# akashsengupta1997/STRAPS-3DHumanShapePose

Hardware: AMD Instinct MI355X
Metric: bodies/sec (higher is better)
Workload: dtype fp32 (encoder convolutions as exact bf16x3 operand splits (six bf16 products per term); in-step SMPL blend contraction and skinning as 3-product fp16 splits (fp16x3_lbs: 22-bit operands); fp32 accumulate throughout)

## Files before the change

straps-3dhumanshapepose_amd/csrc/elementwise.hip:

```cpp
#include "common.h"

namespace {

__global__ __launch_bounds__(256) void pack_krsc_kernel(const float* __restrict__ src, float* __restrict__ dst, int O, int C, int R, int S) {
    const long long i = (long long)blockIdx.x * 256 + threadIdx.x;
    const long long n = (long long)O * C * R * S;
    if (i >= n) return;
    const int c = (int)(i % C);
    long long t = i / C;
    const int s = (int)(t % S); t /= S;
    const int r = (int)(t % R);
    const int o = (int)(t / R);
    dst[i] = src[(((long long)o * C + c) * R + r) * S + s];
}

__global__ __launch_bounds__(256) void pack_crsk_flip_kernel(const float* __restrict__ src, float* __restrict__ dst, int O, int C, int R, int S) {
    const long long i = (long long)blockIdx.x * 256 + threadIdx.x;
    const long long n = (long long)O * C * R * S;
    if (i >= n) return;
    const int o = (int)(i % O);
    long long t = i / O;
    const int s = (int)(t % S); t /= S;
    const int r = (int)(t % R);
    const int c = (int)(t / R);
// ... 145 lines not shown
                const f32x4 v = *reinterpret_cast<const f32x4*>(x + (((long long)b * H + hi) * W + wi) * C + c4 * 4);
                m[0] = fmaxf(m[0], v[0]); m[1] = fmaxf(m[1], v[1]); m[2] = fmaxf(m[2], v[2]); m[3] = fmaxf(m[3], v[3]);
            }
        }
        *reinterpret_cast<f32x4*>(y + i * 4) = m;
    }
}

__global__ __launch_bounds__(256) void gap_kernel(const float* __restrict__ x, float* __restrict__ y, int B, int HW, int C) {
    const long long i = (long long)blockIdx.x * 256 + threadIdx.x;
    if (i >= (long long)B * C) return;
    const int c = (int)(i % C);
    const long long b = i / C;
    const float* p = x + b * HW * C + c;
    float s = 0.f;
    for (int k = 0; k < HW; ++k) s += p[(long long)k * C];
    y[i] = s / (float)HW;
}

__global__ __launch_bounds__(256) void bn_stats_finalize_kernel(const float* __restrict__ part, int nblocks, int C, double count,
                                                               const float* __restrict__ gamma, const float* __restrict__ beta, float eps,
                                                               float momentum, float* __restrict__ rmean, float* __restrict__ rvar,
                                                               float* __restrict__ scale, float* __restrict__ shift,
                                                               float* __restrict__ smean, float* __restrict__ sinv) {
    int c;
    double s1, s2;
    if (bn_partials_sum4(part, nblocks, C, s1, s2, c)) {
        const double mean = s1 / count;
        double var = s2 / count - mean * mean;
        if (var < 0.0) var = 0.0;
        const float inv = (float)(1.0 / sqrt(var + (double)eps));
// ... 193 lines not shown
```

straps-3dhumanshapepose_amd/csrc/smpl_bwd.hip:

```cpp
#include "common.h"
#include "rodrigues.h"

namespace {

constexpr int KP = STRAPS_SMPL_KP, KG = KP / 8, NT = STRAPS_SMPL_TILES, NV = STRAPS_SMPL_V, NROUNDS = NT / 4;
constexpr int BT = 32, AS = 292, SS = 193;
constexpr int NJS = STRAPS_SMPL_NPICK + STRAPS_SMPL_NEXTRA;

__global__ __launch_bounds__(256, 1) STRAPS_NO_PACKED_FP32 void smpl_verts_bwd_kernel(straps_smpl_model_t m, const float* __restrict__ F,
                                                                const float* __restrict__ Amat, const float* __restrict__ dverts,
                                                                const float* __restrict__ djoints, float* __restrict__ dFp,
                                                                float* __restrict__ dAp, long long B, int rounds_per_chunk) {
    extern __shared__ __attribute__((aligned(16))) float smem[];
    float* As_ = smem;
    float* stage = As_ + BT * AS;

    const int tid = threadIdx.x, lane = tid & 63, wave = tid >> 6;
    const int h = lane >> 5, bl = lane & 31;
    const int chunk = blockIdx.x;
    const long long b0 = (long long)blockIdx.y * BT;
    const int nb = (int)((B - b0) < BT ? (B - b0) : BT);

    for (int i = tid; i < BT * 72; i += 256) {
        const int b = i / 72, q = i % 72;
        f32x4 v = {0.f, 0.f, 0.f, 0.f};
        if (b < nb) v = *reinterpret_cast<const f32x4*>(Amat + (b0 + b) * 288 + q * 4);
        *reinterpret_cast<f32x4*>(As_ + b * AS + q * 4) = v;
    }
    __syncthreads();

    const int round0 = chunk * rounds_per_chunk;
    const int round1 = min(round0 + rounds_per_chunk, NROUNDS);
    const f32x4* __restrict__ blend = reinterpret_cast<const f32x4*>(m.blend_frag);
    const f32x4* __restrict__ blend_t = reinterpret_cast<const f32x4*>(m.blend_frag_t);
    float* mystage = stage + wave * BT * SS;
    const int KW = m.skin_k;
    const bool vbody = bl < nb;

    float dacc[3][12];
#pragma unroll
    for (int i = 0; i < 3; ++i)
#pragma unroll
        for (int e = 0; e < 12; ++e) dacc[i][e] = 0.f;
    f32x16 accF[7];
#pragma unroll
    for (int f = 0; f < 7; ++f)
#pragma unroll
        for (int q = 0; q < 16; ++q) accF[f][q] = 0.f;

    for (int rd = round0; rd < round1; ++rd) {
        const int tile = rd * 4 + wave;
        f32x16 ax, ay, az;
#pragma unroll
        for (int r = 0; r < 16; ++r) { ax[r] = 0.f; ay[r] = 0.f; az[r] = 0.f; }
        {
            const f32x4* px = blend + ((long long)(tile * 3 + 0) * KG) * 64 + lane;
            const f32x4* py = px + KG * 64;
            const f32x4* pz = py + KG * 64;
            const float* frow = F + (b0 + (vbody ? bl : 0)) * KP + 4 * h;
            f32x4 cx0 = px[0], cy0 = py[0], cz0 = pz[0];
            f32x4 fn = *reinterpret_cast<const f32x4*>(frow);
#pragma unroll 2
            for (int g = 0; g < KG; ++g) {
                f32x4 nx0 = cx0, ny0 = cy0, nz0 = cz0;
                const f32x4 f0 = vbody ? fn : f32x4{0.f, 0.f, 0.f, 0.f};
                if (g + 1 < KG) {
                    nx0 = px[(g + 1) * 64]; ny0 = py[(g + 1) * 64]; nz0 = pz[(g + 1) * 64];
                    fn = *reinterpret_cast<const f32x4*>(frow + 8 * (g + 1));
                }
#pragma unroll
                for (int e = 0; e < 4; ++e) {
                    ax = mfma32(cx0[e], f0[e], ax);
                    ay = mfma32(cy0[e], f0[e], ay);
                    az = mfma32(cz0[e], f0[e], az);
                }
                cx0 = nx0; cy0 = ny0; cz0 = nz0;
            }
        }
        {
            const int ncol = min(96, (NV - tile * 32) * 3);
            for (int i = lane; i < BT * 96; i += 64) {
                const int b = i / 96, c = i - b * 96;
                float v = 0.f;
                if (dverts && b < nb && c < ncol) v = dverts[(b0 + b) * (long long)(NV * 3) + tile * 96 + c];
                mystage[b * SS + (c / 3) * 6 + (c % 3)] = v;
            }
        }
        __syncthreads();
        if (djoints && h == 0 && vbody) {
            const float* dj = djoints + (b0 + bl) * (STRAPS_SMPL_NJOINTS_OUT * 3) + 72;
            const int e0 = m.jrt_ptr[tile], e1 = m.jrt_ptr[tile + 1];
            for (int e = e0; e < e1; ++e) {
                const int code = m.jrt_code[e];
                const float w = m.jrt_w[e];
                float* sv = mystage + bl * SS + (code >> 8) * 6;
                const float* g = dj + (code & 255) * 3;
                sv[0] = fmaf(w, g[0], sv[0]); sv[1] = fmaf(w, g[1], sv[1]); sv[2] = fmaf(w, g[2], sv[2]);
            }
        }
        __syncthreads();
        {
            const float* Ab = As_ + bl * AS;
#pragma unroll
            for (int r = 0; r < 16; ++r) {
                const int vrow = (r & 3) + 8 * (r >> 2) + 4 * h;
                const int v = tile * 32 + vrow;
                float* sv = mystage + bl * SS + vrow * 6;
                const float gx = sv[0], gy = sv[1], gz = sv[2];
                sv[3] = ax[r]; sv[4] = ay[r]; sv[5] = az[r];
                float t00 = 0.f, t01 = 0.f, t02 = 0.f, t10 = 0.f, t11 = 0.f, t12 = 0.f, t20 = 0.f, t21 = 0.f, t22 = 0.f;
                for (int k = 0; k < KW; ++k) {
                    const float w = m.skin_w[v * KW + k];
                    const int jo = m.skin_j[v * KW + k] * 12;
                    const f32x4 a0 = *reinterpret_cast<const f32x4*>(Ab + jo);
                    const f32x4 a1 = *reinterpret_cast<const f32x4*>(Ab + jo + 4);
                    const f32x4 a2 = *reinterpret_cast<const f32x4*>(Ab + jo + 8);
                    t00 += w * a0[0]; t01 += w * a0[1]; t02 += w * a0[2];
                    t10 += w * a1[0]; t11 += w * a1[1]; t12 += w * a1[2];
                    t20 += w * a2[0]; t21 += w * a2[1]; t22 += w * a2[2];
                }
                ax[r] = t00 * gx + t10 * gy + t20 * gz;
                ay[r] = t01 * gx + t11 * gy + t21 * gz;
                az[r] = t02 * gx + t12 * gy + t22 * gz;
            }
        }
        __syncthreads();
#pragma unroll
        for (int i = 0; i < 3; ++i) {
            const int j = wave + 4 * (2 * i + h);
            const int e0 = m.dj_ptr[rd * 24 + j], e1 = m.dj_ptr[rd * 24 + j + 1];
            for (int e = e0; e < e1; ++e) {
                const int code = m.dj_code[e];
                const float w = m.dj_w[e];
                const float* sv = stage + ((code >> 5) * BT + bl) * SS + (code & 31) * 6;
                const float wx = w * sv[0], wy = w * sv[1], wz = w * sv[2];
                const float x = sv[3], y = sv[4], z = sv[5];
                dacc[i][0] = fmaf(wx, x, dacc[i][0]); dacc[i][1] = fmaf(wx, y, dacc[i][1]); dacc[i][2] = fmaf(wx, z, dacc[i][2]); dacc[i][3] += wx;
                dacc[i][4] = fmaf(wy, x, dacc[i][4]); dacc[i][5] = fmaf(wy, y, dacc[i][5]); dacc[i][6] = fmaf(wy, z, dacc[i][6]); dacc[i][7] += wy;
                dacc[i][8] = fmaf(wz, x, dacc[i][8]); dacc[i][9] = fmaf(wz, y, dacc[i][9]); dacc[i][10] = fmaf(wz, z, dacc[i][10]); dacc[i][11] += wz;
            }
        }
        {
            const f32x4* pt = blend_t + ((long long)tile * 3 * 7 * 4) * 64 + lane;
#pragma unroll
            for (int c = 0; c < 3; ++c) {
#pragma unroll
                for (int f = 0; f < 7; ++f) {
#pragma unroll
                    for (int rq = 0; rq < 4; ++rq) {
                        const f32x4 a = pt[((c * 7 + f) * 4 + rq) * 64];
#pragma unroll
                        for (int e = 0; e < 4; ++e) {
                            const float g = c == 0 ? ax[rq * 4 + e] : (c == 1 ? ay[rq * 4 + e] : az[rq * 4 + e]);
                            accF[f] = mfma32(a[e], g, accF[f]);
                        }
                    }
                }
            }
        }
        __syncthreads();
    }
    {
        __syncthreads();
        float* red = smem;
        if (wave >= 2) {
#pragma unroll
            for (int f = 0; f < 7; ++f)
#pragma unroll
                for (int q = 0; q < 16; ++q) red[(wave - 2) * 7168 + (f * 16 + q) * 64 + lane] = accF[f][q];
        }
        __syncthreads();
// ... 25 lines not shown
#pragma unroll
            for (int q = 0; q < 16; ++q) o[f * 32 + mfma_row(q, lane)] = accF[f][q];
    }
    if (vbody) {
        float* o = dAp + ((long long)chunk * B + b0 + bl) * 288;
#pragma unroll
        for (int i = 0; i < 3; ++i) {
            const int j = wave + 4 * (2 * i + h);
#pragma unroll
            for (int e = 0; e < 12; ++e) o[j * 12 + e] = dacc[i][e];
        }
    }
}

__device__ __forceinline__ float lane_get(float value, int src) { return __shfl(value, src, 64); }
template <bool AA>
__global__ __launch_bounds__(256) STRAPS_NO_PACKED_FP32 void smpl_pose_bwd_kernel(straps_smpl_model_t m, const float* __restrict__ betas,
                                                            const float* __restrict__ rotmats, const float* __restrict__ dFp,
                                                            const float* __restrict__ dAp, const float* __restrict__ djoints,
                                                            float* __restrict__ dbetas, float* __restrict__ drot, long long B,
                                                            int chunks, const float* __restrict__ aa, float* __restrict__ daa) {
    const int lane = threadIdx.x & 63;
    const int j = lane & 31;
    const int base = lane & 32;
    const long long body = ((long long)blockIdx.x * 256 + threadIdx.x) >> 5;
    const bool vb = body < B;
    const bool vj = j < 24;
    const long long bb = vb ? body : 0;
    const int jj = vj ? j : 0;

// ... 35 lines not shown
#pragma unroll
            for (int r = 0; r < 3; ++r) {
                const float p0 = P[r * 4 + 0], p1 = P[r * 4 + 1], p2 = P[r * 4 + 2];
                PR[r * 3 + 0] = p0; PR[r * 3 + 1] = p1; PR[r * 3 + 2] = p2;
                G[r * 4 + 0] = p0 * R[0] + p1 * R[3] + p2 * R[6];
                G[r * 4 + 1] = p0 * R[1] + p1 * R[4] + p2 * R[7];
                G[r * 4 + 2] = p0 * R[2] + p1 * R[5] + p2 * R[8];
                G[r * 4 + 3] = p0 * rel[0] + p1 * rel[1] + p2 * rel[2] + P[r * 4 + 3];
            }
        }
    }
    float gA[12];
#pragma unroll
    for (int e = 0; e < 12; ++e) gA[e] = 0.f;
    if (vb && vj)
        for (int c = 0; c < chunks; ++c) {
            const float* p = dAp + (((long long)c * B + body) * 24 + j) * 12;
#pragma unroll
            for (int e = 0; e < 12; ++e) gA[e] += p[e];
        }
    float gGR[9], gGt[3], gJ[3];
#pragma unroll
    for (int r = 0; r < 3; ++r) {
        const float gat = gA[r * 4 + 3];
        gGR[r * 3 + 0] = gA[r * 4 + 0] - gat * J[0];
        gGR[r * 3 + 1] = gA[r * 4 + 1] - gat * J[1];
        gGR[r * 3 + 2] = gA[r * 4 + 2] - gat * J[2];
        gGt[r] = gat + ((vb && vj && djoints) ? djoints[(body * STRAPS_SMPL_NJOINTS_OUT + j) * 3 + r] : 0.f);
    }
#pragma unroll
    for (int c = 0; c < 3; ++c) gJ[c] = -(G[0 * 4 + c] * gA[3] + G[1 * 4 + c] * gA[7] + G[2 * 4 + c] * gA[11]);

    int child[3];
#pragma unroll
// ... 34 lines not shown
#pragma unroll
                for (int e = 0; e < 9; ++e) gGR[e] += in[e];
#pragma unroll
                for (int c = 0; c < 3; ++c) { gGt[c] += in[9 + c]; gJ[c] += in[12 + c]; }
            }
        }
    }
    if (j == 0) {
#pragma unroll
        for (int e = 0; e < 9; ++e) gR[e] = gGR[e];
#pragma unroll
        for (int c = 0; c < 3; ++c) gJ[c] += gGt[c];
    }
    float gbeta_direct = 0.f;
    if (vb && vj) {
        for (int c = 0; c < chunks; ++c) {
            const float* p = dFp + ((long long)c * B + body) * KP;
            if (j >= 1) {
#pragma unroll
                for (int e = 0; e < 9; ++e) gR[e] += p[11 + (j - 1) * 9 + e];
            }
            if (j < 10) gbeta_direct += p[1 + j];
        }
        if (!AA || drot) {
#pragma unroll
            for (int e = 0; e < 9; ++e) drot[(body * 24 + j) * 9 + e] = gR[e];
        }
        if constexpr (AA) {
            float ox, oy, oz;
            const float* r = aa + (body * 24 + j) * 3;
            straps_rodrigues_bwd_one(r[0], r[1], r[2], gR, ox, oy, oz);
            float* o = daa + (body * 24 + j) * 3;
            o[0] = ox; o[1] = oy; o[2] = oz;
        }
    }
#pragma unroll
    for (int l = 0; l < 10; ++l) {
// ... 25 lines not shown

namespace {
template <bool AA>
int smpl_bwd_launch(const straps_smpl_model_t* model, const float* betas, const float* rotmats, const float* aa, const float* dverts,
                    const float* djoints, float* dbetas, float* drotmats, float* daa, void* workspace, long long batch, int chunks,
                    void* stream) {
    hipStream_t st = (hipStream_t)stream;
    const int rpc = resolve_rpc(batch, chunks);
    const int nch = (NROUNDS + rpc - 1) / rpc;
    float* F = (float*)workspace;
    float* Amat = F + batch * KP;
    float* dFp = Amat + batch * 288;
    float* dAp = dFp + (long long)nch * batch * KP;
    int rc = straps_smpl_launch_pose(model, betas, rotmats, F, Amat, nullptr, batch, st);
    if (rc != STRAPS_OK) return rc;
    const size_t lds = (size_t)(BT * AS + 4 * BT * SS) * sizeof(float);
    STRAPS_RAISE_LDS((smpl_verts_bwd_kernel), lds, "smpl_verts_bwd_kernel");
    const long long btiles = (batch + BT - 1) / BT;
    if (btiles > 65535) { straps_set_error("straps_smpl_bwd: batch %lld exceeds one launch; split it", batch); return STRAPS_EUNSUPPORTED; }
    hipLaunchKernelGGL(smpl_verts_bwd_kernel, dim3(nch, (unsigned)btiles), dim3(256), lds, st, *model, F, Amat, dverts, djoints, dFp, dAp, batch, rpc);
    STRAPS_CHECK_LAUNCH("smpl_verts_bwd_kernel");
    hipLaunchKernelGGL(smpl_pose_bwd_kernel<AA>, dim3((unsigned)((batch * 32 + 255) / 256)), dim3(256), 0, st, *model, betas, rotmats, dFp, dAp,
                       djoints, dbetas, drotmats, batch, nch, aa, daa);
    STRAPS_CHECK_LAUNCH("smpl_pose_bwd_kernel");
    return STRAPS_OK;
}
}

extern "C" int straps_smpl_bwd(const straps_smpl_model_t* model, const float* betas, const float* rotmats, const float* dverts,
                               const float* djoints, float* dbetas, float* drotmats, void* workspace, long long batch, int chunks,
                               void* stream) {
// ... 18 lines not shown
```

straps-3dhumanshapepose_amd/csrc/train.hip:

```cpp
#include <math.h>

#include "common.h"

namespace {

__constant__ int c_coco[17] = {24, 26, 25, 28, 27, 16, 17, 18, 19, 20, 21, 1, 2, 4, 5, 7, 8};
__constant__ int c_h36m14[14] = {73 + 6, 73 + 5, 73 + 4, 73 + 1, 73 + 2, 73 + 3, 73 + 16, 73 + 15, 73 + 14, 73 + 11, 73 + 12, 73 + 13, 73 + 8, 73 + 10};

__device__ __forceinline__ float heat_value(int x, int y, int jx, int jy, int WH, int size, float step, float two_var) {
    if (!(jx > -size && jy > -size && jx < WH - 1 + size && jy < WH - 1 + size)) return 0.f;
    const int hx0 = max(0, jx - size), hx1 = min(WH - 1, jx + size);
    const int hy0 = max(0, jy - size), hy1 = min(WH - 1, jy + size);
    if (!(x >= hx0 && x < hx1 && y >= hy0 && y < hy1)) return 0.f;
    const int gx = x - hx0 + max(0, size - jx), gy = y - hy0 + max(0, size - jy);
    const float fs = (float)size;
    const float lx = gx < size ? -fs + step * gx : fs - step * (2 * size - 1 - gx);
    const float ly = gy < size ? -fs + step * gy : fs - step * (2 * size - 1 - gy);
    const float d = sqrtf(lx * lx + ly * ly);
    return expf(-(d * d / two_var));
}

__global__ __launch_bounds__(256) void build_proxy_kernel(const float* __restrict__ seg, const float* __restrict__ j2d,
                                                          float* __restrict__ out, int B, int NJ, int WH, int size, float step, float two_var) {
    const int plane = blockIdx.y;
// ... 69 lines not shown
            }
        }
#pragma unroll
        for (int r = 0; r < 4; ++r)
            if (y0 + r < WH) {
                *reinterpret_cast<f32x4*>(o + (y0 + r) * WH + x0) = v[r];
                nz = nz || v[r][0] != 0.f || v[r][1] != 0.f || v[r][2] != 0.f || v[r][3] != 0.f;
            }
    }
    const unsigned long long m = __ballot(nz);
    if (lane == 0) mask[word] = (unsigned)(m | (m >> 32));
}

constexpr int NVB = 1024;

__global__ __launch_bounds__(256) void loss_verts_partial_kernel(const float* __restrict__ p, const float* __restrict__ t, long long n,
                                                                 float* __restrict__ part) {
    __shared__ float red[4];
    float s = 0.f;
    for (long long i = (long long)blockIdx.x * 256 + threadIdx.x; i < n; i += (long long)gridDim.x * 256) {
        const float d = p[i] - t[i];
        s = fmaf(d, d, s);
    }
#pragma unroll
    for (int o = 32; o > 0; o >>= 1) s += __shfl_xor(s, o, 64);
    if ((threadIdx.x & 63) == 0) red[threadIdx.x >> 6] = s;
    __syncthreads();
    if (threadIdx.x == 0) part[blockIdx.x] = (red[0] + red[1]) + (red[2] + red[3]);
}

__device__ __forceinline__ bool joint_visible(float x, float y, float wh) { return !(x > wh || y > wh || x < 0.f || y < 0.f); }

__global__ __launch_bounds__(256) void loss_heads_kernel(const float* __restrict__ joints, const float* __restrict__ est, int ld_est,
                                                         const float* __restrict__ prot, const float* __restrict__ tj2d,
                                                         const float* __restrict__ tj3d, const float* __restrict__ tshape,
                                                         const float* __restrict__ trot, float* __restrict__ body_sums, long long B,
                                                         float wh) {
    const long long b = (long long)blockIdx.x * 256 + threadIdx.x;
    if (b >= B) return;
    const float* J = joints + b * 270;
    const float* e = est + b * ld_est;
    const float s = e[0], tx = e[1], ty = e[2];
    float sq2 = 0.f, nvis = 0.f, sq3 = 0.f, sqs = 0.f, sqr = 0.f;
    for (int k = 0; k < 17; ++k) {
        const float lx = tj2d[(b * 17 + k) * 2 + 0], ly = tj2d[(b * 17 + k) * 2 + 1];
        if (joint_visible(lx, ly, wh)) {
            const float* pj = J + c_coco[k] * 3;
            const float u = s * (pj[0] + tx), v = s * (pj[1] + ty);
            const float du = u - ((2.0f * lx) / wh - 1.0f), dv = v - ((2.0f * ly) / wh - 1.0f);
            sq2 += du * du + dv * dv;
            nvis += 1.f;
        }
    }
    for (int k = 0; k < 14; ++k) {
        const float* pj = J + c_h36m14[k] * 3;
        const float* tj = tj3d + (b * 14 + k) * 3;
        for (int c = 0; c < 3; ++c) { const float d = pj[c] - tj[c]; sq3 += d * d; }
    }
    for (int l = 0; l < 10; ++l) { const float d = e[147 + l] - tshape[b * 10 + l]; sqs += d * d; }
    for (int q = 0; q < 216; ++q) { const float d = prot[b * 216 + q] - trot[b * 216 + q]; sqr += d * d; }
    float* o = body_sums + b * 8;
    o[0] = sq2; o[1] = nvis; o[2] = sq3; o[3] = sqs; o[4] = sqr;
}

__global__ __launch_bounds__(256) void loss_finalize_kernel(const float* __restrict__ vpart, const float* __restrict__ body_sums,
                                                            const float* __restrict__ log_vars, float* __restrict__ loss_out,
                                                            float* __restrict__ dlogvar, float* __restrict__ coef, long long B,
                                                            const float* __restrict__ j2d_count, float count_scale) {
    __shared__ double red[256][6];
    double a[6] = {0, 0, 0, 0, 0, 0};
    for (int i = threadIdx.x; i < NVB; i += 256) a[0] += (double)vpart[i];
    for (long long b = threadIdx.x; b < B; b += 256) {
        const float* o = body_sums + b * 8;
        a[1] += o[0]; a[2] += o[1]; a[3] += o[2]; a[4] += o[3]; a[5] += o[4];
    }
    for (int q = 0; q < 6; ++q) red[threadIdx.x][q] = a[q];
    __syncthreads();
    if (threadIdx.x == 0) {
        double t[6] = {0, 0, 0, 0, 0, 0};
        for (int i = 0; i < 256; ++i)
            for (int q = 0; q < 6; ++q) t[q] += red[i][q];
        const double nvis = t[2];
        const double n2 = j2d_count ? (double)j2d_count[0] * (double)count_scale : nvis;
        const double cnt[5] = {(double)B * 20670.0, n2 * 2.0, (double)B * 42.0, (double)B * 10.0, (double)B * 216.0};
        const double sq[5] = {t[0], t[1], t[3], t[4], t[5]};
        double total = 0.0;
        for (int k = 0; k < 5; ++k) {
            const double mse = sq[k] / cnt[k];
            const double s = (double)log_vars[k];
            const double w = exp(-s);
            loss_out[1 + k] = (float)(mse * w);
            loss_out[6 + k] = (float)mse;
            total += mse * w + s;
            dlogvar[k] = (float)(-mse * w + 1.0);
            coef[k] = (float)(2.0 * w / cnt[k]);
        }
        loss_out[0] = (float)total;
        loss_out[11] = (float)nvis;
    }
}

__global__ __launch_bounds__(256) void loss_grad_verts_kernel(const float* __restrict__ p, const float* __restrict__ t,
                                                              const float* __restrict__ coef, float* __restrict__ g, long long n) {
    const float c = coef[0];
    for (long long i = (long long)blockIdx.x * 256 + threadIdx.x; i < n; i += (long long)gridDim.x * 256) g[i] = c * (p[i] - t[i]);
}

__global__ __launch_bounds__(64) STRAPS_NO_PACKED_FP32 void loss_grad_heads_kernel(const float* __restrict__ joints, const float* __restrict__ est, int ld_est,
                                                             const float* __restrict__ prot, const float* __restrict__ tj2d,
                                                             const float* __restrict__ tj3d, const float* __restrict__ tshape,
                                                             const float* __restrict__ trot, const float* __restrict__ coef,
                                                             float* __restrict__ djoints, float* __restrict__ dest,
                                                             float* __restrict__ drot, long long B, float wh) {
    const long long b = blockIdx.x;
    const int lane = threadIdx.x;
    const float* J = joints + b * 270;
    const float* e = est + b * ld_est;
    float* dJ = djoints + b * 270;
    float* dE = dest + b * ld_est;
    const float c2 = coef[1], c3 = coef[2], cs = coef[3], cr = coef[4];
    for (int i = lane; i < 270; i += 64) dJ[i] = 0.f;
    for (int i = lane; i < ld_est; i += 64) dE[i] = (i >= 147 && i < 157) ? cs * (e[i] - tshape[b * 10 + i - 147]) : 0.f;
    for (int i = lane; i < 216; i += 64) drot[b * 216 + i] = cr * (prot[b * 216 + i] - trot[b * 216 + i]);
    __builtin_amdgcn_s_waitcnt(0);
    __syncthreads();
    const float s = e[0], tx = e[1], ty = e[2];
    float gs = 0.f, gtx = 0.f, gty = 0.f;
    if (lane < 17) {
        const float lx = tj2d[(b * 17 + lane) * 2 + 0], ly = tj2d[(b * 17 + lane) * 2 + 1];
        if (joint_visible(lx, ly, wh)) {
            const float* pj = J + c_coco[lane] * 3;
            const float u = s * (pj[0] + tx), v = s * (pj[1] + ty);
            const float du = c2 * (u - ((2.0f * lx) / wh - 1.0f)), dv = c2 * (v - ((2.0f * ly) / wh - 1.0f));
            dJ[c_coco[lane] * 3 + 0] = du * s;
            dJ[c_coco[lane] * 3 + 1] = dv * s;
            gs = du * (pj[0] + tx) + dv * (pj[1] + ty);
            gtx = du * s;
            gty = dv * s;
        }
    } else if (lane >= 32 && lane < 46) {
// ... 105 lines not shown
                                      const float* tgt_rot, const float* log_vars, float* loss_out, float* dverts, float* djoints,
                                      float* dest, float* drot, float* dlogvar, void* workspace, long long batch, int img_wh,
                                      const float* j2d_count_global, float count_scale, void* stream) {
    STRAPS_REQUIRE(pred_verts && pred_joints && est && pred_rot && tgt_verts && tgt_joints2d && tgt_joints3d && tgt_shape && tgt_rot &&
                       log_vars && loss_out && workspace,
                   "straps_loss_fwd_bwd: null pointer");
    STRAPS_REQUIRE(batch > 0 && ld_est >= 157, "straps_loss_fwd_bwd: bad shape batch=%lld ld_est=%d", batch, ld_est);
    const bool want_grad = dverts || djoints || dest || drot;
    STRAPS_REQUIRE(!want_grad || (dverts && djoints && dest && drot && dlogvar), "straps_loss_fwd_bwd: give all gradient outputs or none");
    hipStream_t st = (hipStream_t)stream;
    float* vpart = (float*)workspace;
    float* body = vpart + NVB;
    float* coef = body + batch * 8;
    float* dlv = dlogvar ? dlogvar : coef + 8;
    const long long nv = batch * 20670LL;
    hipLaunchKernelGGL(loss_verts_partial_kernel, dim3(NVB), dim3(256), 0, st, pred_verts, tgt_verts, nv, vpart);
    STRAPS_CHECK_LAUNCH("loss_verts_partial_kernel");
    hipLaunchKernelGGL(loss_heads_kernel, dim3((unsigned)((batch + 255) / 256)), dim3(256), 0, st, pred_joints, est, ld_est, pred_rot,
                       tgt_joints2d, tgt_joints3d, tgt_shape, tgt_rot, body, batch, (float)img_wh);
    STRAPS_CHECK_LAUNCH("loss_heads_kernel");
    hipLaunchKernelGGL(loss_finalize_kernel, dim3(1), dim3(256), 0, st, vpart, body, log_vars, loss_out, dlv, coef, batch, j2d_count_global, count_scale);
    STRAPS_CHECK_LAUNCH("loss_finalize_kernel");
    if (want_grad) {
        hipLaunchKernelGGL(loss_grad_verts_kernel, dim3(capped_grid(nv)), dim3(256), 0, st, pred_verts, tgt_verts, coef, dverts, nv);
        STRAPS_CHECK_LAUNCH("loss_grad_verts_kernel");
        hipLaunchKernelGGL(loss_grad_heads_kernel, dim3((unsigned)batch), dim3(64), 0, st, pred_joints, est, ld_est, pred_rot, tgt_joints2d,
                           tgt_joints3d, tgt_shape, tgt_rot, coef, djoints, dest, drot, batch, (float)img_wh);
        STRAPS_CHECK_LAUNCH("loss_grad_heads_kernel");
    }
    return STRAPS_OK;
}

extern "C" int straps_adam_step(float* params, const float* grads, float* exp_avg, float* exp_avg_sq, long long n, int step, float lr,
                                float beta1, float beta2, float eps, float grad_scale, const long long* step_dev, void* stream) {
    STRAPS_REQUIRE(params && grads && exp_avg && exp_avg_sq && n > 0 && (step >= 1 || step_dev), "straps_adam_step: bad arguments");
    if (step < 1) step = 1;
    const double bc1 = 1.0 - pow((double)beta1, (double)step);
    const double bc2 = 1.0 - pow((double)beta2, (double)step);
    hipLaunchKernelGGL(adam_kernel, dim3(capped_grid(n)), dim3(256), 0, (hipStream_t)stream, params, grads, exp_avg, exp_avg_sq, n, beta1, beta2,
                       eps, (float)((double)lr / bc1), (float)(1.0 / sqrt(bc2)), grad_scale, lr, step_dev);
    STRAPS_CHECK_LAUNCH("adam_kernel");
    return STRAPS_OK;
}
// ... 94 lines not shown
```

Before: 7968.

## Software-pipeline SMPL backward loads, stage djoints in LDS, and fuse loss kernels

```diff
diff --git a/straps-3dhumanshapepose_amd/csrc/elementwise.hip b/straps-3dhumanshapepose_amd/csrc/elementwise.hip
--- a/straps-3dhumanshapepose_amd/csrc/elementwise.hip
+++ b/straps-3dhumanshapepose_amd/csrc/elementwise.hip
@@ -183,7 +183,16 @@
     const long long b = i / C;
     const float* p = x + b * HW * C + c;
     float s = 0.f;
-    for (int k = 0; k < HW; ++k) s += p[(long long)k * C];
+    int k = 0;
+    for (; k + 16 <= HW; k += 16) {
+        float v[16];
+#pragma unroll
+        for (int u = 0; u < 16; ++u) v[u] = p[(long long)(k + u) * C];
+        __builtin_amdgcn_sched_barrier(0);
+#pragma unroll
+        for (int u = 0; u < 16; ++u) s += v[u];
+    }
+    for (; k < HW; ++k) s += p[(long long)k * C];
     y[i] = s / (float)HW;
 }
 
diff --git a/straps-3dhumanshapepose_amd/csrc/smpl_bwd.hip b/straps-3dhumanshapepose_amd/csrc/smpl_bwd.hip
--- a/straps-3dhumanshapepose_amd/csrc/smpl_bwd.hip
+++ b/straps-3dhumanshapepose_amd/csrc/smpl_bwd.hip
@@ -6,6 +6,33 @@
 constexpr int KP = STRAPS_SMPL_KP, KG = KP / 8, NT = STRAPS_SMPL_TILES, NV = STRAPS_SMPL_V, NROUNDS = NT / 4;
 constexpr int BT = 32, AS = 292, SS = 193;
 constexpr int NJS = STRAPS_SMPL_NPICK + STRAPS_SMPL_NEXTRA;
+
+__device__ __forceinline__ void sched_fence() { __builtin_amdgcn_sched_barrier(0); }
+__device__ __forceinline__ float lane_bcast(float v, int l) { return __builtin_bit_cast(float, __builtin_amdgcn_readlane(__builtin_bit_cast(int, v), l)); }
+template <int N>
+__device__ __forceinline__ void owner_sums(const int (&oc)[N], const float (&ow)[N], const float* stage, int bl, float (&d)[12]) {
+#pragma unroll
+    for (int u = 0; u < N; ++u) {
+        const int code = oc[u];
+        const float w = ow[u];
+        const float* sv = stage + ((code >> 5) * BT + bl) * SS + (code & 31) * 6;
+        const float wx = w * sv[0], wy = w * sv[1], wz = w * sv[2];
+        const float x = sv[3], y = sv[4], z = sv[5];
+        d[0] = fmaf(wx, x, d[0]); d[1] = fmaf(wx, y, d[1]); d[2] = fmaf(wx, z, d[2]); d[3] += wx;
+        d[4] = fmaf(wy, x, d[4]); d[5] = fmaf(wy, y, d[5]); d[6] = fmaf(wy, z, d[6]); d[7] += wy;
+        d[8] = fmaf(wz, x, d[8]); d[9] = fmaf(wz, y, d[9]); d[10] = fmaf(wz, z, d[10]); d[11] += wz;
+    }
+}
+template <int N>
+__device__ __forceinline__ void owner_entries(const int* __restrict__ codes, const float* __restrict__ ws, const float* stage, int bl, float (&d)[12]) {
+    int oc[N];
+    float ow[N];
+#pragma unroll
+    for (int u = 0; u < N; ++u) { oc[u] = codes[u]; ow[u] = ws[u]; }
+    sched_fence();
+    owner_sums<N>(oc, ow, stage, bl, d);
+}
+constexpr int RING1 = 3, RING4 = 8, DJS = NJS * 3 + 1;
 
 __global__ __launch_bounds__(256, 1) STRAPS_NO_PACKED_FP32 void smpl_verts_bwd_kernel(straps_smpl_model_t m, const float* __restrict__ F,
                                                                 const float* __restrict__ Amat, const float* __restrict__ dverts,
@@ -14,18 +41,42 @@
     extern __shared__ __attribute__((aligned(16))) float smem[];
     float* As_ = smem;
     float* stage = As_ + BT * AS;
-
-    const int tid = threadIdx.x, lane = tid & 63, wave = tid >> 6;
+    float* djs = stage + 4 * BT * SS;
+
+    const int tid = threadIdx.x, lane = tid & 63, wave = __builtin_amdgcn_readfirstlane(tid >> 6);
     const int h = lane >> 5, bl = lane & 31;
     const int chunk = blockIdx.x;
     const long long b0 = (long long)blockIdx.y * BT;
     const int nb = (int)((B - b0) < BT ? (B - b0) : BT);
 
-    for (int i = tid; i < BT * 72; i += 256) {
-        const int b = i / 72, q = i % 72;
-        f32x4 v = {0.f, 0.f, 0.f, 0.f};
-        if (b < nb) v = *reinterpret_cast<const f32x4*>(Amat + (b0 + b) * 288 + q * 4);
-        *reinterpret_cast<f32x4*>(As_ + b * AS + q * 4) = v;
+    {
+        f32x4 av[9];
+        float jv[25];
+#pragma unroll
+        for (int t = 0; t < 9; ++t) {
+            const int i = tid + t * 256, b = i / 72, q = i % 72;
+            av[t] = *reinterpret_cast<const f32x4*>(Amat + (b0 + (b < nb ? b : 0)) * 288 + q * 4);
+        }
+        if (djoints) {
+#pragma unroll
+            for (int t = 0; t < 25; ++t) {
+                const int i = min(tid + t * 256, BT * NJS * 3 - 1), b = i / (NJS * 3), q = i % (NJS * 3);
+                jv[t] = djoints[(b0 + (b < nb ? b : 0)) * (STRAPS_SMPL_NJOINTS_OUT * 3) + 72 + q];
+            }
+        }
+        sched_fence();
+#pragma unroll
+        for (int t = 0; t < 9; ++t) {
+            const int i = tid + t * 256, b = i / 72, q = i % 72;
+            *reinterpret_cast<f32x4*>(As_ + b * AS + q * 4) = b < nb ? av[t] : f32x4{0.f, 0.f, 0.f, 0.f};
+        }
+        if (djoints) {
+#pragma unroll
+            for (int t = 0; t < 25; ++t) {
+                const int i = tid + t * 256, b = i / (NJS * 3), q = i % (NJS * 3);
+                if (i < BT * NJS * 3) djs[b * DJS + q] = jv[t];
+            }
+        }
     }
     __syncthreads();
 
@@ -36,6 +87,15 @@
     float* mystage = stage + wave * BT * SS;
     const int KW = m.skin_k;
     const bool vbody = bl < nb;
+    const bool dv_pairs = dverts && (reinterpret_cast<unsigned long long>(dverts) & 7) == 0;
+
+    int so[3][2];
+#pragma unroll
+    for (int q = 0; q < 3; ++q) {
+        const int c = 32 * q + 2 * (lane & 15);
+        so[q][0] = (lane >> 4) * SS + (c / 3) * 6 + (c % 3);
+        so[q][1] = (lane >> 4) * SS + ((c + 1) / 3) * 6 + ((c + 1) % 3);
+    }
 
     float dacc[3][12];
 #pragma unroll
@@ -50,6 +110,15 @@
 
     for (int rd = round0; rd < round1; ++rd) {
         const int tile = rd * 4 + wave;
+        const int ncol = min(96, (NV - tile * 32) * 3);
+        const int je0 = m.jrt_ptr[tile], je1 = m.jrt_ptr[tile + 1];
+        int oe0[3], oe1[3];
+#pragma unroll
+        for (int i = 0; i < 3; ++i) {
+            const int j = wave + 4 * (2 * i + h);
+            oe0[i] = m.dj_ptr[rd * 24 + j]; oe1[i] = m.dj_ptr[rd * 24 + j + 1];
+        }
+        sched_fence();
         f32x16 ax, ay, az;
 #pragma unroll
         for (int r = 0; r < 16; ++r) { ax[r] = 0.f; ay[r] = 0.f; az[r] = 0.f; }
@@ -57,28 +126,53 @@
             const f32x4* px = blend + ((long long)(tile * 3 + 0) * KG) * 64 + lane;
             const f32x4* py = px + KG * 64;
             const f32x4* pz = py + KG * 64;
-            const float* frow = F + (b0 + (vbody ? bl : 0)) * KP + 4 * h;
-            f32x4 cx0 = px[0], cy0 = py[0], cz0 = pz[0];
-            f32x4 fn = *reinterpret_cast<const f32x4*>(frow);
-#pragma unroll 2
+            int fo = (vbody ? bl : 0) * KP + 4 * h;
+            asm volatile("" : "+v"(fo));
+            const float* frow = F + b0 * KP + fo;
+            f32x4 rx[RING1], ry[RING1], rz[RING1], rf[RING1];
+#pragma unroll
+            for (int s = 0; s < RING1; ++s) {
+                rx[s] = px[s * 64]; ry[s] = py[s * 64]; rz[s] = pz[s * 64];
+                rf[s] = *reinterpret_cast<const f32x4*>(frow + 8 * s);
+            }
+            sched_fence();
+#pragma unroll
             for (int g = 0; g < KG; ++g) {
-                f32x4 nx0 = cx0, ny0 = cy0, nz0 = cz0;
-                const f32x4 f0 = vbody ? fn : f32x4{0.f, 0.f, 0.f, 0.f};
-                if (g + 1 < KG) {
-                    nx0 = px[(g + 1) * 64]; ny0 = py[(g + 1) * 64]; nz0 = pz[(g + 1) * 64];
-                    fn = *reinterpret_cast<const f32x4*>(frow + 8 * (g + 1));
-                }
+                const int s = g % RING1;
+                const f32x4 cx0 = rx[s], cy0 = ry[s], cz0 = rz[s];
+                const f32x4 f0 = vbody ? rf[s] : f32x4{0.f, 0.f, 0.f, 0.f};
 #pragma unroll
                 for (int e = 0; e < 4; ++e) {
                     ax = mfma32(cx0[e], f0[e], ax);
                     ay = mfma32(cy0[e], f0[e], ay);
                     az = mfma32(cz0[e], f0[e], az);
                 }
-                cx0 = nx0; cy0 = ny0; cz0 = nz0;
-            }
-        }
-        {
-            const int ncol = min(96, (NV - tile * 32) * 3);
+                if (g + RING1 < KG) {
+                    rx[s] = px[(g + RING1) * 64]; ry[s] = py[(g + RING1) * 64]; rz[s] = pz[(g + RING1) * 64];
+                    rf[s] = *reinterpret_cast<const f32x4*>(frow + 8 * (g + RING1));
+                }
+                sched_fence();
+            }
+        }
+        if (dv_pairs) {
+            f32x2 dvp[24];
+            int sb = lane >> 4;
+            asm volatile("" : "+v"(sb));
+#pragma unroll
+            for (int t = 0; t < 24; ++t) {
+                const int b = 4 * (t / 3) + sb, c = 32 * (t % 3) + 2 * (lane & 15);
+                const bool ok = b < nb && c < ncol;
+                dvp[t] = *reinterpret_cast<const f32x2*>(dverts + (b0 + (ok ? b : 0)) * (long long)(NV * 3) + tile * 96 + (ok ? c : 0));
+            }
+            sched_fence();
+#pragma unroll
+            for (int t = 0; t < 24; ++t) {
+                const int b = 4 * (t / 3) + (lane >> 4), c = 32 * (t % 3) + 2 * (lane & 15);
+                const bool ok = b < nb && c < ncol;
+                mystage[so[t % 3][0] + (t / 3) * 4 * SS] = ok ? dvp[t][0] : 0.f;
+                mystage[so[t % 3][1] + (t / 3) * 4 * SS] = ok ? dvp[t][1] : 0.f;
+            }
+        } else {
             for (int i = lane; i < BT * 96; i += 64) {
                 const int b = i / 96, c = i - b * 96;
                 float v = 0.f;
@@ -86,16 +180,37 @@
                 mystage[b * SS + (c / 3) * 6 + (c % 3)] = v;
             }
         }
-        __syncthreads();
-        if (djoints && h == 0 && vbody) {
-            const float* dj = djoints + (b0 + bl) * (STRAPS_SMPL_NJOINTS_OUT * 3) + 72;
-            const int e0 = m.jrt_ptr[tile], e1 = m.jrt_ptr[tile + 1];
-            for (int e = e0; e < e1; ++e) {
-                const int code = m.jrt_code[e];
-                const float w = m.jrt_w[e];
-                float* sv = mystage + bl * SS + (code >> 8) * 6;
-                const float* g = dj + (code & 255) * 3;
-                sv[0] = fmaf(w, g[0], sv[0]); sv[1] = fmaf(w, g[1], sv[1]); sv[2] = fmaf(w, g[2], sv[2]);
+        float skw0 = 0.f, skw1 = 0.f;
+        int skj0 = 0, skj1 = 0;
+        if (KW == 4) {
+            skw0 = m.skin_w[tile * 128 + lane]; skw1 = m.skin_w[tile * 128 + 64 + lane];
+            skj0 = m.skin_j[tile * 128 + lane]; skj1 = m.skin_j[tile * 128 + 64 + lane];
+        }
+        const f32x4* pt = blend_t + ((long long)tile * 3 * 7 * 4) * 64 + lane;
+        f32x4 ring[RING4];
+#pragma unroll
+        for (int s = 0; s < RING4; ++s) ring[s] = pt[s * 64];
+        int jcode = 0;
+        float jw = 0.f;
+        if (djoints && je0 + lane < je1) { jcode = m.jrt_code[je0 + lane]; jw = m.jrt_w[je0 + lane]; }
+        sched_fence();
+        __syncthreads();
+        if (djoints) {
+            for (int eb = je0; eb < je1; eb += 64) {
+                if (eb != je0) {
+                    jcode = 0; jw = 0.f;
+                    if (eb + lane < je1) { jcode = m.jrt_code[eb + lane]; jw = m.jrt_w[eb + lane]; }
+                }
+                const int ne = min(64, je1 - eb);
+                for (int i = 0; i < ne; ++i) {
+                    const int code = __builtin_amdgcn_readlane(jcode, i);
+                    const float w = lane_bcast(jw, i);
+                    if (h == 0 && vbody) {
+                        float* sv = mystage + bl * SS + (code >> 8) * 6;
+                        const float* g = djs + bl * DJS + (code & 255) * 3;
+                        sv[0] = fmaf(w, g[0], sv[0]); sv[1] = fmaf(w, g[1], sv[1]); sv[2] = fmaf(w, g[2], sv[2]);
+                    }
+                }
             }
         }
         __syncthreads();
@@ -109,15 +224,30 @@
                 const float gx = sv[0], gy = sv[1], gz = sv[2];
                 sv[3] = ax[r]; sv[4] = ay[r]; sv[5] = az[r];
                 float t00 = 0.f, t01 = 0.f, t02 = 0.f, t10 = 0.f, t11 = 0.f, t12 = 0.f, t20 = 0.f, t21 = 0.f, t22 = 0.f;
-                for (int k = 0; k < KW; ++k) {
-                    const float w = m.skin_w[v * KW + k];
-                    const int jo = m.skin_j[v * KW + k] * 12;
-                    const f32x4 a0 = *reinterpret_cast<const f32x4*>(Ab + jo);
-                    const f32x4 a1 = *reinterpret_cast<const f32x4*>(Ab + jo + 4);
-                    const f32x4 a2 = *reinterpret_cast<const f32x4*>(Ab + jo + 8);
-                    t00 += w * a0[0]; t01 += w * a0[1]; t02 += w * a0[2];
-                    t10 += w * a1[0]; t11 += w * a1[1]; t12 += w * a1[2];
-                    t20 += w * a2[0]; t21 += w * a2[1]; t22 += w * a2[2];
+                if (KW == 4) {
+#pragma unroll
+                    for (int k = 0; k < 4; ++k) {
+                        const int src = (4 * vrow + k) & 63;
+                        const float w = __shfl((r >> 2) < 2 ? skw0 : skw1, src, 64);
+                        const int jo = __shfl((r >> 2) < 2 ? skj0 : skj1, src, 64) * 12;
+                        const f32x4 a0 = *reinterpret_cast<const f32x4*>(Ab + jo);
+                        const f32x4 a1 = *reinterpret_cast<const f32x4*>(Ab + jo + 4);
+                        const f32x4 a2 = *reinterpret_cast<const f32x4*>(Ab + jo + 8);
+                        t00 += w * a0[0]; t01 += w * a0[1]; t02 += w * a0[2];
+                        t10 += w * a1[0]; t11 += w * a1[1]; t12 += w * a1[2];
+                        t20 += w * a2[0]; t21 += w * a2[1]; t22 += w * a2[2];
+                    }
+                } else {
+                    for (int k = 0; k < KW; ++k) {
+                        const float w = m.skin_w[v * KW + k];
+                        const int jo = m.skin_j[v * KW + k] * 12;
+                        const f32x4 a0 = *reinterpret_cast<const f32x4*>(Ab + jo);
+                        const f32x4 a1 = *reinterpret_cast<const f32x4*>(Ab + jo + 4);
+                        const f32x4 a2 = *reinterpret_cast<const f32x4*>(Ab + jo + 8);
+                        t00 += w * a0[0]; t01 += w * a0[1]; t02 += w * a0[2];
+                        t10 += w * a1[0]; t11 += w * a1[1]; t12 += w * a1[2];
+                        t20 += w * a2[0]; t21 += w * a2[1]; t22 += w * a2[2];
+                    }
                 }
                 ax[r] = t00 * gx + t10 * gy + t20 * gz;
                 ay[r] = t01 * gx + t11 * gy + t21 * gz;
@@ -127,34 +257,45 @@
         __syncthreads();
 #pragma unroll
         for (int i = 0; i < 3; ++i) {
-            const int j = wave + 4 * (2 * i + h);
-            const int e0 = m.dj_ptr[rd * 24 + j], e1 = m.dj_ptr[rd * 24 + j + 1];
-            for (int e = e0; e < e1; ++e) {
-                const int code = m.dj_code[e];
-                const float w = m.dj_w[e];
-                const float* sv = stage + ((code >> 5) * BT + bl) * SS + (code & 31) * 6;
-                const float wx = w * sv[0], wy = w * sv[1], wz = w * sv[2];
-                const float x = sv[3], y = sv[4], z = sv[5];
-                dacc[i][0] = fmaf(wx, x, dacc[i][0]); dacc[i][1] = fmaf(wx, y, dacc[i][1]); dacc[i][2] = fmaf(wx, z, dacc[i][2]); dacc[i][3] += wx;
-                dacc[i][4] = fmaf(wy, x, dacc[i][4]); dacc[i][5] = fmaf(wy, y, dacc[i][5]); dacc[i][6] = fmaf(wy, z, dacc[i][6]); dacc[i][7] += wy;
-                dacc[i][8] = fmaf(wz, x, dacc[i][8]); dacc[i][9] = fmaf(wz, y, dacc[i][9]); dacc[i][10] = fmaf(wz, z, dacc[i][10]); dacc[i][11] += wz;
-            }
-        }
-        {
-            const f32x4* pt = blend_t + ((long long)tile * 3 * 7 * 4) * 64 + lane;
-#pragma unroll
-            for (int c = 0; c < 3; ++c) {
-#pragma unroll
-                for (int f = 0; f < 7; ++f) {
-#pragma unroll
-                    for (int rq = 0; rq < 4; ++rq) {
-                        const f32x4 a = pt[((c * 7 + f) * 4 + rq) * 64];
-#pragma unroll
-                        for (int e = 0; e < 4; ++e) {
-                            const float g = c == 0 ? ax[rq * 4 + e] : (c == 1 ? ay[rq * 4 + e] : az[rq * 4 + e]);
-                            accF[f] = mfma32(a[e], g, accF[f]);
-                        }
+            int e = oe0[i];
+            const int e1 = oe1[i];
+            if (e + 8 <= e1) {
+                int nc[8];
+                float nw[8];
+#pragma unroll
+                for (int u = 0; u < 8; ++u) { nc[u] = m.dj_code[e + u]; nw[u] = m.dj_w[e + u]; }
+                for (; e + 8 <= e1; e += 8) {
+                    int oc[8];
+                    float ow[8];
+#pragma unroll
+                    for (int u = 0; u < 8; ++u) { oc[u] = nc[u]; ow[u] = nw[u]; }
+#pragma unroll
+                    for (int u = 0; u < 8; ++u) { const int en = min(e + 8 + u, e1 - 1); nc[u] = m.dj_code[en]; nw[u] = m.dj_w[en]; }
+                    sched_fence();
+                    owner_sums<8>(oc, ow, stage, bl, dacc[i]);
+                    sched_fence();
+                }
+            }
+            if (e + 4 <= e1) { owner_entries<4>(m.dj_code + e, m.dj_w + e, stage, bl, dacc[i]); e += 4; }
+            if (e + 2 <= e1) { owner_entries<2>(m.dj_code + e, m.dj_w + e, stage, bl, dacc[i]); e += 2; }
+            if (e < e1) owner_entries<1>(m.dj_code + e, m.dj_w + e, stage, bl, dacc[i]);
+        }
+        sched_fence();
+#pragma unroll
+        for (int c = 0; c < 3; ++c) {
+#pragma unroll
+            for (int f = 0; f < 7; ++f) {
+#pragma unroll
+                for (int rq = 0; rq < 4; ++rq) {
+                    const int q = (c * 7 + f) * 4 + rq;
+                    const f32x4 a = ring[q % RING4];
+#pragma unroll
+                    for (int e = 0; e < 4; ++e) {
+                        const float g = c == 0 ? ax[rq * 4 + e] : (c == 1 ? ay[rq * 4 + e] : az[rq * 4 + e]);
+                        accF[f] = mfma32(a[e], g, accF[f]);
                     }
+                    if (q + RING4 < 84) ring[q % RING4] = pt[(q + RING4) * 64];
+                    sched_fence();
                 }
             }
         }
@@ -210,6 +351,8 @@
 }
 
 __device__ __forceinline__ float lane_get(float value, int src) { return __shfl(value, src, 64); }
+constexpr int PB = 9;
+__device__ __forceinline__ void pose_sched_fence() { __builtin_amdgcn_sched_barrier(0); }
 template <bool AA>
 __global__ __launch_bounds__(256) STRAPS_NO_PACKED_FP32 void smpl_pose_bwd_kernel(straps_smpl_model_t m, const float* __restrict__ betas,
                                                             const float* __restrict__ rotmats, const float* __restrict__ dFp,
@@ -275,10 +418,21 @@
 #pragma unroll
     for (int e = 0; e < 12; ++e) gA[e] = 0.f;
     if (vb && vj)
-        for (int c = 0; c < chunks; ++c) {
-            const float* p = dAp + (((long long)c * B + body) * 24 + j) * 12;
-#pragma unroll
-            for (int e = 0; e < 12; ++e) gA[e] += p[e];
+        for (int c0 = 0; c0 < chunks; c0 += PB) {
+            float buf[PB][12];
+#pragma unroll
+            for (int u = 0; u < PB; ++u) {
+                const float* p = dAp + (((long long)min(c0 + u, chunks - 1) * B + body) * 24 + j) * 12;
+#pragma unroll
+                for (int e = 0; e < 12; ++e) buf[u][e] = p[e];
+            }
+            pose_sched_fence();
+#pragma unroll
+            for (int u = 0; u < PB; ++u)
+                if (c0 + u < chunks) {
+#pragma unroll
+                    for (int e = 0; e < 12; ++e) gA[e] += buf[u][e];
+                }
         }
     float gGR[9], gGt[3], gJ[3];
 #pragma unroll
@@ -343,13 +497,26 @@
     }
     float gbeta_direct = 0.f;
     if (vb && vj) {
-        for (int c = 0; c < chunks; ++c) {
-            const float* p = dFp + ((long long)c * B + body) * KP;
-            if (j >= 1) {
-#pragma unroll
-                for (int e = 0; e < 9; ++e) gR[e] += p[11 + (j - 1) * 9 + e];
-            }
-            if (j < 10) gbeta_direct += p[1 + j];
+        const int offR = 11 + (j >= 1 ? j - 1 : 0) * 9, offB = 1 + (j < 10 ? j : 0);
+        for (int c0 = 0; c0 < chunks; c0 += PB) {
+            float bufR[PB][9], bufB[PB];
+#pragma unroll
+            for (int u = 0; u < PB; ++u) {
+                const float* p = dFp + ((long long)min(c0 + u, chunks - 1) * B + body) * KP;
+#pragma unroll
+                for (int e = 0; e < 9; ++e) bufR[u][e] = p[offR + e];
+                bufB[u] = p[offB];
+            }
+            pose_sched_fence();
+#pragma unroll
+            for (int u = 0; u < PB; ++u)
+                if (c0 + u < chunks) {
+                    if (j >= 1) {
+#pragma unroll
+                        for (int e = 0; e < 9; ++e) gR[e] += bufR[u][e];
+                    }
+                    if (j < 10) gbeta_direct += bufB[u];
+                }
         }
         if (!AA || drot) {
 #pragma unroll
@@ -405,7 +572,7 @@
     float* dAp = dFp + (long long)nch * batch * KP;
     int rc = straps_smpl_launch_pose(model, betas, rotmats, F, Amat, nullptr, batch, st);
     if (rc != STRAPS_OK) return rc;
-    const size_t lds = (size_t)(BT * AS + 4 * BT * SS) * sizeof(float);
+    const size_t lds = (size_t)(BT * AS + 4 * BT * SS + BT * DJS) * sizeof(float);
     STRAPS_RAISE_LDS((smpl_verts_bwd_kernel), lds, "smpl_verts_bwd_kernel");
     const long long btiles = (batch + BT - 1) / BT;
     if (btiles > 65535) { straps_set_error("straps_smpl_bwd: batch %lld exceeds one launch; split it", batch); return STRAPS_EUNSUPPORTED; }
diff --git a/straps-3dhumanshapepose_amd/csrc/train.hip b/straps-3dhumanshapepose_amd/csrc/train.hip
--- a/straps-3dhumanshapepose_amd/csrc/train.hip
+++ b/straps-3dhumanshapepose_amd/csrc/train.hip
@@ -107,36 +107,59 @@
 
 constexpr int NVB = 1024;
 
-__global__ __launch_bounds__(256) void loss_verts_partial_kernel(const float* __restrict__ p, const float* __restrict__ t, long long n,
-                                                                 float* __restrict__ part) {
+__device__ __forceinline__ bool joint_visible(float x, float y, float wh) { return !(x > wh || y > wh || x < 0.f || y < 0.f); }
+
+constexpr int HB_J = 0, HB_E = 272, HB_T2 = 432, HB_T3 = 468, HB_TS = 512, HB_PR = 524, HB_TR = 740, HB_ROW = 956;
+
+__device__ __forceinline__ void wave_copy(float* dst, const float* __restrict__ src, int n, int lane) {
+    for (int i = lane; i < n; i += 64) dst[i] = src[i];
+}
+
+__global__ __launch_bounds__(256) void loss_sums_kernel(const float* __restrict__ p, const float* __restrict__ t, long long n, float* __restrict__ part,
+                                                        const float* __restrict__ joints, const float* __restrict__ est, int ld_est,
+                                                        const float* __restrict__ prot, const float* __restrict__ tj2d,
+                                                        const float* __restrict__ tj3d, const float* __restrict__ tshape,
+                                                        const float* __restrict__ trot, float* __restrict__ body_sums, long long B, float wh) {
     __shared__ float red[4];
-    float s = 0.f;
-    for (long long i = (long long)blockIdx.x * 256 + threadIdx.x; i < n; i += (long long)gridDim.x * 256) {
-        const float d = p[i] - t[i];
-        s = fmaf(d, d, s);
-    }
-#pragma unroll
-    for (int o = 32; o > 0; o >>= 1) s += __shfl_xor(s, o, 64);
-    if ((threadIdx.x & 63) == 0) red[threadIdx.x >> 6] = s;
+    __shared__ float rows[4][HB_ROW];
+    if (blockIdx.x < NVB) {
+        float s = 0.f;
+        for (long long i = (long long)blockIdx.x * 256 + threadIdx.x; i < n; i += (long long)NVB * 256) {
+            const float d = p[i] - t[i];
+            s = fmaf(d, d, s);
+        }
+#pragma unroll
+        for (int o = 32; o > 0; o >>= 1) s += __shfl_xor(s, o, 64);
+        if ((threadIdx.x & 63) == 0) red[threadIdx.x >> 6] = s;
+        __syncthreads();
+        if (threadIdx.x == 0) part[blockIdx.x] = (red[0] + red[1]) + (red[2] + red[3]);
+        return;
+    }
+    const int lane = threadIdx.x & 63, wave = threadIdx.x >> 6;
+    const long long b = (long long)(blockIdx.x - NVB) * 4 + wave;
+    float* row = rows[wave];
+    if (b < B) {
+        wave_copy(row + HB_J, joints + b * 270, 270, lane);
+        wave_copy(row + HB_E, est + b * ld_est, 157, lane);
+        wave_copy(row + HB_T2, tj2d + b * 34, 34, lane);
+        wave_copy(row + HB_T3, tj3d + b * 42, 42, lane);
+        wave_copy(row + HB_TS, tshape + b * 10, 10, lane);
+        wave_copy(row + HB_PR, prot + b * 216, 216, lane);
+        wave_copy(row + HB_TR, trot + b * 216, 216, lane);
+    }
     __syncthreads();
-    if (threadIdx.x == 0) part[blockIdx.x] = (red[0] + red[1]) + (red[2] + red[3]);
-}
-
-__device__ __forceinline__ bool joint_visible(float x, float y, float wh) { return !(x > wh || y > wh || x < 0.f || y < 0.f); }
-
-__global__ __launch_bounds__(256) void loss_heads_kernel(const float* __restrict__ joints, const float* __restrict__ est, int ld_est,
-                                                         const float* __restrict__ prot, const float* __restrict__ tj2d,
-                                                         const float* __restrict__ tj3d, const float* __restrict__ tshape,
-                                                         const float* __restrict__ trot, float* __restrict__ body_sums, long long B,
-                                                         float wh) {
-    const long long b = (long long)blockIdx.x * 256 + threadIdx.x;
-    if (b >= B) return;
-    const float* J = joints + b * 270;
-    const float* e = est + b * ld_est;
+    if (b >= B || lane != 0) return;
+    const float* J = row + HB_J;
+    const float* e = row + HB_E;
+    const float* l2 = row + HB_T2;
+    const float* l3 = row + HB_T3;
+    const float* ls = row + HB_TS;
+    const float* pr = row + HB_PR;
+    const float* tr = row + HB_TR;
     const float s = e[0], tx = e[1], ty = e[2];
     float sq2 = 0.f, nvis = 0.f, sq3 = 0.f, sqs = 0.f, sqr = 0.f;
     for (int k = 0; k < 17; ++k) {
-        const float lx = tj2d[(b * 17 + k) * 2 + 0], ly = tj2d[(b * 17 + k) * 2 + 1];
+        const float lx = l2[k * 2 + 0], ly = l2[k * 2 + 1];
         if (joint_visible(lx, ly, wh)) {
             const float* pj = J + c_coco[k] * 3;
             const float u = s * (pj[0] + tx), v = s * (pj[1] + ty);
@@ -147,11 +170,11 @@
     }
     for (int k = 0; k < 14; ++k) {
         const float* pj = J + c_h36m14[k] * 3;
-        const float* tj = tj3d + (b * 14 + k) * 3;
+        const float* tj = l3 + k * 3;
         for (int c = 0; c < 3; ++c) { const float d = pj[c] - tj[c]; sq3 += d * d; }
     }
-    for (int l = 0; l < 10; ++l) { const float d = e[147 + l] - tshape[b * 10 + l]; sqs += d * d; }
-    for (int q = 0; q < 216; ++q) { const float d = prot[b * 216 + q] - trot[b * 216 + q]; sqr += d * d; }
+    for (int l = 0; l < 10; ++l) { const float d = e[147 + l] - ls[l]; sqs += d * d; }
+    for (int q = 0; q < 216; ++q) { const float d = pr[q] - tr[q]; sqr += d * d; }
     float* o = body_sums + b * 8;
     o[0] = sq2; o[1] = nvis; o[2] = sq3; o[3] = sqs; o[4] = sqr;
 }
@@ -162,7 +185,13 @@
                                                             const float* __restrict__ j2d_count, float count_scale) {
     __shared__ double red[256][6];
     double a[6] = {0, 0, 0, 0, 0, 0};
-    for (int i = threadIdx.x; i < NVB; i += 256) a[0] += (double)vpart[i];
+    {
+        float v[NVB / 256];
+#pragma unroll
+        for (int u = 0; u < NVB / 256; ++u) v[u] = vpart[threadIdx.x + u * 256];
+#pragma unroll
+        for (int u = 0; u < NVB / 256; ++u) a[0] += (double)v[u];
+    }
     for (long long b = threadIdx.x; b < B; b += 256) {
         const float* o = body_sums + b * 8;
         a[1] += o[0]; a[2] += o[1]; a[3] += o[2]; a[4] += o[3]; a[5] += o[4];
@@ -171,8 +200,18 @@
     __syncthreads();
     if (threadIdx.x == 0) {
         double t[6] = {0, 0, 0, 0, 0, 0};
-        for (int i = 0; i < 256; ++i)
-            for (int q = 0; q < 6; ++q) t[q] += red[i][q];
+        for (int i0 = 0; i0 < 256; i0 += 8) {
+            double v[8][6];
+#pragma unroll
+            for (int u = 0; u < 8; ++u)
+#pragma unroll
+                for (int q = 0; q < 6; ++q) v[u][q] = red[i0 + u][q];
+            __builtin_amdgcn_sched_barrier(0);
+#pragma unroll
+            for (int u = 0; u < 8; ++u)
+#pragma unroll
+                for (int q = 0; q < 6; ++q) t[q] += v[u][q];
+        }
         const double nvis = t[2];
         const double n2 = j2d_count ? (double)j2d_count[0] * (double)count_scale : nvis;
         const double cnt[5] = {(double)B * 20670.0, n2 * 2.0, (double)B * 42.0, (double)B * 10.0, (double)B * 216.0};
@@ -193,30 +232,37 @@
     }
 }
 
-__global__ __launch_bounds__(256) void loss_grad_verts_kernel(const float* __restrict__ p, const float* __restrict__ t,
-                                                              const float* __restrict__ coef, float* __restrict__ g, long long n) {
-    const float c = coef[0];
-    for (long long i = (long long)blockIdx.x * 256 + threadIdx.x; i < n; i += (long long)gridDim.x * 256) g[i] = c * (p[i] - t[i]);
-}
-
-__global__ __launch_bounds__(64) STRAPS_NO_PACKED_FP32 void loss_grad_heads_kernel(const float* __restrict__ joints, const float* __restrict__ est, int ld_est,
-                                                             const float* __restrict__ prot, const float* __restrict__ tj2d,
-                                                             const float* __restrict__ tj3d, const float* __restrict__ tshape,
-                                                             const float* __restrict__ trot, const float* __restrict__ coef,
-                                                             float* __restrict__ djoints, float* __restrict__ dest,
-                                                             float* __restrict__ drot, long long B, float wh) {
-    const long long b = blockIdx.x;
-    const int lane = threadIdx.x;
-    const float* J = joints + b * 270;
-    const float* e = est + b * ld_est;
-    float* dJ = djoints + b * 270;
-    float* dE = dest + b * ld_est;
+__global__ __launch_bounds__(256) STRAPS_NO_PACKED_FP32 void loss_grads_kernel(const float* __restrict__ p, const float* __restrict__ t, float* __restrict__ g,
+                                                        long long n, int head_blocks,
+                                                        const float* __restrict__ joints, const float* __restrict__ est, int ld_est,
+                                                        const float* __restrict__ prot, const float* __restrict__ tj2d,
+                                                        const float* __restrict__ tj3d, const float* __restrict__ tshape,
+                                                        const float* __restrict__ trot, const float* __restrict__ coef,
+                                                        float* __restrict__ djoints, float* __restrict__ dest,
+                                                        float* __restrict__ drot, long long B, float wh) {
+    if ((int)blockIdx.x >= head_blocks) {
+        const float c = coef[0];
+        const long long nblk = (long long)gridDim.x - head_blocks;
+        for (long long i = (long long)(blockIdx.x - head_blocks) * 256 + threadIdx.x; i < n; i += nblk * 256) g[i] = c * (p[i] - t[i]);
+        return;
+    }
+    const long long b = (long long)blockIdx.x * 4 + (threadIdx.x >> 6);
+    const int lane = threadIdx.x & 63;
+    const bool vb = b < B;
+    const long long bb = vb ? b : 0;
+    const float* J = joints + bb * 270;
+    const float* e = est + bb * ld_est;
+    float* dJ = djoints + bb * 270;
+    float* dE = dest + bb * ld_est;
     const float c2 = coef[1], c3 = coef[2], cs = coef[3], cr = coef[4];
-    for (int i = lane; i < 270; i += 64) dJ[i] = 0.f;
-    for (int i = lane; i < ld_est; i += 64) dE[i] = (i >= 147 && i < 157) ? cs * (e[i] - tshape[b * 10 + i - 147]) : 0.f;
-    for (int i = lane; i < 216; i += 64) drot[b * 216 + i] = cr * (prot[b * 216 + i] - trot[b * 216 + i]);
+    if (vb) {
+        for (int i = lane; i < 270; i += 64) dJ[i] = 0.f;
+        for (int i = lane; i < ld_est; i += 64) dE[i] = (i >= 147 && i < 157) ? cs * (e[i] - tshape[b * 10 + i - 147]) : 0.f;
+        for (int i = lane; i < 216; i += 64) drot[b * 216 + i] = cr * (prot[b * 216 + i] - trot[b * 216 + i]);
+    }
     __builtin_amdgcn_s_waitcnt(0);
     __syncthreads();
+    if (!vb) return;
     const float s = e[0], tx = e[1], ty = e[2];
     float gs = 0.f, gtx = 0.f, gty = 0.f;
     if (lane < 17) {
@@ -352,19 +398,18 @@
     float* coef = body + batch * 8;
     float* dlv = dlogvar ? dlogvar : coef + 8;
     const long long nv = batch * 20670LL;
-    hipLaunchKernelGGL(loss_verts_partial_kernel, dim3(NVB), dim3(256), 0, st, pred_verts, tgt_verts, nv, vpart);
-    STRAPS_CHECK_LAUNCH("loss_verts_partial_kernel");
-    hipLaunchKernelGGL(loss_heads_kernel, dim3((unsigned)((batch + 255) / 256)), dim3(256), 0, st, pred_joints, est, ld_est, pred_rot,
+    const unsigned head_blocks = (unsigned)((batch + 3) / 4);
+    STRAPS_REQUIRE(batch <= (1LL << 31), "straps_loss_fwd_bwd: batch %lld exceeds one launch", batch);
+    hipLaunchKernelGGL(loss_sums_kernel, dim3(NVB + head_blocks), dim3(256), 0, st, pred_verts, tgt_verts, nv, vpart, pred_joints, est, ld_est, pred_rot,
                        tgt_joints2d, tgt_joints3d, tgt_shape, tgt_rot, body, batch, (float)img_wh);
-    STRAPS_CHECK_LAUNCH("loss_heads_kernel");
+    STRAPS_CHECK_LAUNCH("loss_sums_kernel");
     hipLaunchKernelGGL(loss_finalize_kernel, dim3(1), dim3(256), 0, st, vpart, body, log_vars, loss_out, dlv, coef, batch, j2d_count_global, count_scale);
     STRAPS_CHECK_LAUNCH("loss_finalize_kernel");
     if (want_grad) {
-        hipLaunchKernelGGL(loss_grad_verts_kernel, dim3(capped_grid(nv)), dim3(256), 0, st, pred_verts, tgt_verts, coef, dverts, nv);
-        STRAPS_CHECK_LAUNCH("loss_grad_verts_kernel");
-        hipLaunchKernelGGL(loss_grad_heads_kernel, dim3((unsigned)batch), dim3(64), 0, st, pred_joints, est, ld_est, pred_rot, tgt_joints2d,
-                           tgt_joints3d, tgt_shape, tgt_rot, coef, djoints, dest, drot, batch, (float)img_wh);
-        STRAPS_CHECK_LAUNCH("loss_grad_heads_kernel");
+        hipLaunchKernelGGL(loss_grads_kernel, dim3(head_blocks + capped_grid(nv)), dim3(256), 0, st, pred_verts, tgt_verts, dverts, nv, (int)head_blocks,
+                           pred_joints, est, ld_est, pred_rot, tgt_joints2d, tgt_joints3d, tgt_shape, tgt_rot, coef, djoints, dest, drot, batch,
+                           (float)img_wh);
+        STRAPS_CHECK_LAUNCH("loss_grads_kernel");
     }
     return STRAPS_OK;
 }
```

After: 8074, median of 6. +1.3%, better.
